# ngrabaskas/Torch-Automatic-Distributed-Neural-Network

Measured on AMD Instinct MI355X. Metric: samples/sec whole-node ResNet-50 DP + GPT-2 PP at 1/2/4/8 MI355X; scaling eff, higher is better.
Workload: dtype bf16

## Files before the change

madnn/models/resnet.py:

```python
from __future__ import annotations

import os
from typing import List, Optional, Type

import torch
from torch import nn

from ..nn.conv import FusedConv2d
from ..nn.norm import FusedBatchNorm2d as BN
from ..nn.norm import FusedGlobalAvgPool2d, FusedMaxPool2d
from ..ops import (batch_norm_add_bn_relu, bn_relu_conv1x1, bn_relu_conv1x1_epi_supported,
                   bn_relu_conv3x3, conv1x1_route,
                   bn_relu_conv3x3_supported, bn_relu_maxpool, bn_relu_maxpool_supported)

_FORK_DS = os.environ.get("MADNN_FORK_DOWNSAMPLE", "1") != "0"
_DUAL_BN = os.environ.get("MADNN_DUAL_BN", "1") != "0"
_DS_SUB = os.environ.get("MADNN_DS_SUB", "1") != "0"


def conv3x3(cin, cout, stride=1, groups=1, dilation=1):
    return FusedConv2d(cin, cout, 3, stride=stride, padding=dilation, groups=groups, bias=False, dilation=dilation)


def conv1x1(cin, cout, stride=1):
    return FusedConv2d(cin, cout, 1, stride=stride, bias=False)


class BasicBlock(nn.Module):
    expansion = 1

    def __init__(self, inplanes, planes, stride=1, downsample=None):
        super().__init__()
        self.conv1 = conv3x3(inplanes, planes, stride)
        self.bn1 = BN(planes)
        self.conv2 = conv3x3(planes, planes)
        self.bn2 = BN(planes)
        self.downsample = downsample

    def forward(self, x):
        idt = x if self.downsample is None else self.downsample(x)
        y, st = self.conv1(x, stats=True)
        out = self.bn1(y, relu=True, stats=st)
        y, st = self.conv2(out, stats=True)
        return self.bn2(y, residual=idt, relu=True, stats=st)


class Bottleneck(nn.Module):
    expansion = 4

    def __init__(self, inplanes, planes, stride=1, downsample=None):
        super().__init__()
        self.conv1 = conv1x1(inplanes, planes)
        self.bn1 = BN(planes)
        self.conv2 = conv3x3(planes, planes, stride)
        self.bn2 = BN(planes)
        self.conv3 = conv1x1(planes, planes * 4)
        self.bn3 = BN(planes * 4)
        self.downsample = downsample

    def forward(self, x):
        if self.downsample is None:
            y, st, idt = self.conv1(x, stats=True, fork=True)
            if isinstance(idt, torch.Tensor) and isinstance(self.bn3, BN) and self.conv1._k9(x) \
                    and conv1x1_route(x.size(1), self.conv1.weight.size(0))[1] == "k9":
                idt._madnn_defer_mask = True
        elif _FORK_DS:
            dual = self._dual_bn()
            sub = dual and _DS_SUB and isinstance(x, torch.Tensor) and self.downsample[0].subsampled_ok()
            y, st, xf = self.conv1(x, stats=True, fork=2 if sub else True)
            if dual:
                yd, std = (self.downsample[0].forward_subsampled(xf, stats=True) if sub
                           else self.downsample[0](xf, stats=True))
                y, st = self._bn1_conv2(y, st)
                y, st = self._bn2_conv3(y, st)
                return batch_norm_add_bn_relu(y, yd, self.bn3, self.downsample[1], st, std)
            idt = self.downsample(xf)
        else:
            idt = self.downsample(x)
            y, st = self.conv1(x, stats=True)
        y, st = self._bn1_conv2(y, st)
        y, st = self._bn2_conv3(y, st)
        return self.bn3(y, residual=idt, relu=True, stats=st)

    def _bn1_conv2(self, y, st):
        if isinstance(y, torch.Tensor) and isinstance(self.bn1, BN) and isinstance(self.conv2, FusedConv2d) \
                and self.conv2._k13(y) \
                and bn_relu_conv3x3_supported(y, self.bn1, self.conv2.weight):
            return bn_relu_conv3x3(y, self.bn1, self.conv2.weight, stats_in=st, stats=True)
        out = self.bn1(y, relu=True, stats=st)
        return self.conv2(out, stats=True)

    def _bn2_conv3(self, y, st):
        if isinstance(y, torch.Tensor) and isinstance(self.bn2, BN) and isinstance(self.conv3, FusedConv2d) \
                and self.conv3._k9(y) and bn_relu_conv1x1_epi_supported(y, self.bn2, self.conv3.weight):
            return bn_relu_conv1x1(y, self.bn2, self.conv3.weight, stats_in=st, stats=True)
        out = self.bn2(y, relu=True, stats=st)
        return self.conv3(out, stats=True)

    def _dual_bn(self) -> bool:
        ds = self.downsample
        return (_DUAL_BN and isinstance(ds, nn.Sequential) and len(ds) == 2
                and isinstance(ds[0], FusedConv2d) and isinstance(ds[1], BN) and isinstance(self.bn3, BN))


class ResNet(nn.Module):
# ... 80 lines not shown
```

madnn/ops/__init__.py:

```python
from __future__ import annotations

import os
import threading
from pathlib import Path
from typing import Optional, Sequence

import torch
import torch.nn.functional as F

from . import reference

HERE = Path(__file__).resolve().parent
_KERNELS = HERE / "_madnn_kernels.so"
_lock = threading.Lock()
_loaded = {"kernels": False, "error": None}


def kernels_path() -> Path:
    return _KERNELS


class StaleKernelsError(RuntimeError):
    """The in-tree kernel library was built from different sources than the tree holds."""

# ... 188 lines not shown
def _attach(t: torch.Tensor, name: str, value) -> None:
    setattr(t, name, (value, t._version))


def _attached(t: Optional[torch.Tensor], name: str, strict: bool = False):
    if t is None:
        return None
    rec = getattr(t, name, None)
    if rec is None and t._base is not None and t.numel() == t._base.numel():
        rec = getattr(t._base, name, None)
    if rec is None:
        return None
    value, version = rec
    if t._version != version:
        if strict:
            raise RuntimeError(f"madnn: gradient carrying {name} was modified in place after it was produced "
                               "(a second consumer's gradient accumulated into it); disable the deferral "
                               "(MADNN_DEFER_RES_MASK=0) for this model")
        return None
    return value


class _BNFn(torch.autograd.Function):
    @staticmethod
    def forward(ctx, x, weight, bias, residual, running_mean, running_var, nbt, training, momentum, eps, relu, stats):
        y, mean, invstd, scale, shift, mask = torch.ops.madnn.bn_fwd(x, residual, weight, bias, running_mean,
                                                                      running_var, nbt, bool(training),
                                                                      float(momentum), float(eps), bool(relu),
                                                                      stats if training else None)
        ctx.save_for_backward(x, mask, weight, mean, invstd, scale, shift)
        ctx.relu = relu
        ctx.has_res = residual is not None
        ctx.has_w = weight is not None
        ctx.defer = (DEFER_RES_MASK and relu and residual is not None and mask.numel() > 0
                     and getattr(residual, "_madnn_defer_mask", False))
        return y

    @staticmethod
    def backward(ctx, dy):
        x, mask, weight, mean, invstd, scale, shift = ctx.saved_tensors
        need_w = ctx.has_w and (ctx.needs_input_grad[1] or ctx.needs_input_grad[2])
        defer = ctx.defer and dy.dtype == x.dtype and dy.stride() == x.stride()
        dx, dw, db, dres = torch.ops.madnn.bn_bwd(dy, x, mask if mask.numel() else None, ctx.has_res, weight,
                                                  mean, invstd, scale, shift, ctx.relu, need_w, not defer)
        if defer:
            dres = dy.view_as(dy)
# ... 474 lines not shown


def bn_relu_conv1x1(y: torch.Tensor, bn, w: torch.Tensor, *, stats_in: Optional[torch.Tensor] = None,
                    stats: bool = False):
    if bn_relu_conv1x1_epi_supported(y, bn, w):
        _need_native("bn_relu_conv1x1")
        out, part = _BNReluConv1x1EpiFn.apply(y, w, bn.weight, bn.bias, bn, stats_in, stats)
        return (out, part if part.numel() else None) if stats else out
    a = bn(y, relu=True, stats=stats_in) if _is_fused_bn(bn) else torch.relu(bn(y))
    if conv1x1_supported(a, w):
        return conv1x1(a, w, stats=stats)
    out = torch.nn.functional.conv2d(a, w.view(w.size(0), -1, 1, 1)) if a.dim() == 4 else torch.mm(
        a, w.reshape(w.size(0), -1).t())
    return (out, None) if stats else out


def bn_relu_conv1x1_epi_supported(y: torch.Tensor, bn, w: torch.Tensor) -> bool:
    return (_BN_DGRAD_EPI and isinstance(y, torch.Tensor) and bn.training and bn.track_running_stats
            and bn.affine and bn.momentum is not None and bn.weight.dtype == torch.float32
            and conv1x1_supported(y, w) and bn_supported(y, bn.weight)
            and conv1x1_route(y.size(1), w.size(0))[1] == "k9")


class _BNReluMaxPoolFn(torch.autograd.Function):

    @staticmethod
    def forward(ctx, y, bn_w, bn_b, bn, stats_in, p):
        mean, invstd, scale, shift = torch.ops.madnn.bn_coef(y, bn_w, bn_b, bn.running_mean, bn.running_var,
                                                             bn.num_batches_tracked, float(bn.momentum),
                                                             float(bn.eps), stats_in)
        out, arg = torch.ops.madnn.pool_bn_fwd(y, scale, shift, int(p))
        ctx.save_for_backward(y, arg, bn_w, mean, invstd, scale, shift)
        ctx.p = int(p)
        return out

    @staticmethod
    def backward(ctx, dp):
        y, arg, bn_w, mean, invstd, scale, shift = ctx.saved_tensors
        dy, dw, db = torch.ops.madnn.pool_bn_bwd(dp, arg, y, bn_w, mean, invstd, scale, shift, ctx.p)
        return dy, dw, db, None, None, None


def bn_relu_maxpool_supported(y: torch.Tensor, bn, pool) -> bool:
    def pair(v):
        return tuple(v) if isinstance(v, (tuple, list)) else (v, v)
    return (_POOL_BN and isinstance(y, torch.Tensor) and y.device.type == "cuda" and y.dtype == torch.bfloat16 and y.dim() == 4
# ... 806 lines not shown
```

madnn/ops/csrc/binding.cpp:

```cpp
#include <torch/library.h>
#include <ATen/ATen.h>
#include <ATen/hip/impl/HIPGuardImplMasqueradingAsCUDA.h>
#include <ATen/hip/impl/HIPStreamMasqueradingAsCUDA.h>
#include <hip/hip_runtime.h>

#include <vector>

#include "attn.h"

extern "C" {
hipError_t madnn_bucket_pack(void* const*, const int64_t*, const int64_t*, int, void*, int, int, float, hipStream_t);
hipError_t madnn_bucket_unpack(void* const*, const int64_t*, const int64_t*, int, void*, int, int, float, hipStream_t);
hipError_t madnn_flat_scale_cast(const void*, void*, int64_t, int, int, float, hipStream_t);
hipError_t madnn_sgd_step(float*, const void*, int, float*, void*, int, int64_t, float, float, float, float, int, int,
                          float, const float*, hipStream_t);
hipError_t madnn_adam_step(float*, const void*, int, float*, float*, void*, int, int64_t, float, float, float, float,
                           float, int, float, float, float, const float*, hipStream_t);
int madnn_sqnorm_grid(int64_t);
hipError_t madnn_sqnorm_partial(const void*, int, int64_t, float, float*, int, hipStream_t);
hipError_t madnn_norm_finalize(const float*, int, float, float*, hipStream_t);
hipError_t madnn_norm_fwd(const void*, const void*, const void*, const void*, void*, void*, float*, float*, int64_t,
                          int, float, int, int, int, hipStream_t);
int64_t madnn_norm_bwd_workspace(int64_t, int);
hipError_t madnn_norm_bwd(const void*, const void*, const void*, const float*, const float*, const void*, void*, void*,
// ... 53 lines not shown
int64_t madnn_conv1x1_wgrad_ws(int64_t, int64_t, int64_t);
hipError_t madnn_conv1x1_wgrad(const void*, const void*, void*, int, float*, int64_t, int64_t, int64_t, hipStream_t);
hipError_t madnn_bn_coef(const void*, int64_t, int, float, float, const float*, const float*, float*, float*, int64_t*,
                         float*, float*, float*, float*, float*, const float*, int, hipStream_t);
int madnn_stem_supported(int, int);
int madnn_stem_stat_rows(int, int, int);
hipError_t madnn_stem_fwd(const void*, const void*, void*, float*, int, int, int, hipStream_t);
int64_t madnn_stem_wgrad_ws(int, int, int);
hipError_t madnn_stem_wgrad(const void*, const void*, float*, float*, int, int, int, hipStream_t);
int madnn_gemm_supported(int64_t, int64_t, int64_t, int64_t, int64_t);
int madnn_conv3x3_supported(int, int, int, int);
int madnn_conv3x3_stat_rows(int64_t);
hipError_t madnn_conv3x3_fwd(const void*, const void*, void*, float*, int, int, int, int, int, hipStream_t);
int madnn_conv3x3_s2_supported(int, int, int, int);
int madnn_conv3x3_s2_stat_rows(int, int, int);
hipError_t madnn_conv3x3_fwd_s2(const void*, const void*, void*, float*, int, int, int, int, int, hipStream_t);
int64_t madnn_conv3x3_wgrad_ws(int, int, int, int, int);
hipError_t madnn_conv3x3_fwd_bnb(const void*, const void*, void*, float*, const void*, const float*, const float*, int,
                                 int, int, int, int, hipStream_t);
hipError_t madnn_bn_bwd_ext(const void*, const void*, void*, int64_t, int, int, const float*, const float*,
                            const float*, const float*, const float*, float*, float*, float*, const float*, int, float*,
                            hipStream_t);
int madnn_bn_prereduce_floats(int);
hipError_t madnn_conv3x3_wgrad(const void*, const void*, float*, void*, int, int, int, int, int, int, hipStream_t);
hipError_t madnn_linear_fwd(const void*, const void*, const void*, int, const void*, void*, void*, int, int64_t,
                            int64_t, int64_t, hipStream_t);
hipError_t madnn_linear_dgrad(const void*, const void*, const void*, void*, int64_t, int64_t, int64_t, hipStream_t);
int madnn_wgrad_splits(int64_t, int64_t, int64_t);
hipError_t madnn_linear_wgrad4h(const void*, const void*, void*, float*, int, int, int64_t, int64_t, int64_t,
                                hipStream_t);
hipError_t madnn_linear_wgrad4(const void*, const void*, void*, float*, int, int, int64_t, int64_t, int64_t,
                               hipStream_t);
hipError_t madnn_linear_wgrad(const void*, const void*, void*, float*, int, int, int64_t, int64_t, int64_t,
                              hipStream_t);
int madnn_gemmp_supported(int64_t, int64_t, int64_t, int);
hipError_t madnn_linear_fwd_p(const void*, const void*, const void*, int, void*, void*, int, int64_t, int64_t,
                              int64_t, hipStream_t);
hipError_t madnn_linear_dgrad_p(const void*, const void*, const void*, void*, float*, int64_t, int64_t, int64_t, int,
                                hipStream_t);
hipError_t madnn_colsum_finalize(const float*, int, int64_t, void*, int, hipStream_t);
hipError_t madnn_hwq_wait(const int*, int, int64_t, int*, hipStream_t);
hipError_t madnn_hwq_set(int*, int, hipStream_t);
hipError_t madnn_hwq_batch(const int*, const int*, int, int*, int*, int, int64_t, int*, const int*, hipStream_t);
hipError_t madnn_hwq_spin(int64_t, hipStream_t);
}

// ... 468 lines not shown
                         const c10::optional<at::Tensor>& resmask) {
  const int64_t cout = dy.size(1), cin = w.numel() / std::max<int64_t>(cout, 1);
  const int64_t M = conv_rows(dy, cout, "dy");
  conv_check_w(w, cout, cin);
  at::hip::HIPGuardMasqueradingAsCUDA guard(dy.device());
  at::Tensor dx = conv_out_like(dy, cin);
  const bool has_res = res.has_value() && res->defined();
  if (has_res) {
    TORCH_CHECK(conv_rows(*res, cin, "res") == M && res->dim() == dy.dim(), "conv1x1_dgrad: residual layout");
  }
  const bool has_mask = resmask.has_value() && resmask->defined();
  if (has_mask) {
    TORCH_CHECK(has_res && resmask->scalar_type() == at::kByte && resmask->is_contiguous() &&
                    resmask->numel() == M * cin / 8, "conv1x1_dgrad: resmask must be a uint8 bit mask over res");
  }
  check(madnn_conv1x1_dgrad(dy.data_ptr(), w.data_ptr(), dx.data_ptr(), has_res ? res->data_ptr() : nullptr, M, cin,
                            cout, nullptr, nullptr, nullptr, nullptr, cur_stream(dy),
                            has_mask ? resmask->data_ptr<uint8_t>() : nullptr),
        "conv1x1_dgrad");
  return dx;
}

std::tuple<at::Tensor, at::Tensor> conv1x1_dgrad_bnb(const at::Tensor& dy, const at::Tensor& w, const at::Tensor& bny,
                                                     const at::Tensor& scale, const at::Tensor& shift) {
  const int64_t cout = dy.size(1), cin = w.numel() / std::max<int64_t>(cout, 1);
  const int64_t M = conv_rows(dy, cout, "dy");
  conv_check_w(w, cout, cin);
  TORCH_CHECK(conv_rows(bny, cin, "bny") == M && bny.dim() == dy.dim(), "conv1x1_dgrad_bnb: bny layout");
  TORCH_CHECK(scale.numel() == cin && shift.numel() == cin && scale.scalar_type() == at::kFloat &&
                  shift.scalar_type() == at::kFloat && scale.is_contiguous() && shift.is_contiguous(),
              "conv1x1_dgrad_bnb: fp32 [Cin] scale / shift");
  at::hip::HIPGuardMasqueradingAsCUDA guard(dy.device());
  at::Tensor dx = conv_out_like(dy, cin);
  at::Tensor part = at::empty({madnn_conv1x1_dgrad_rows(M, cin, cout), 2, cin}, dy.options().dtype(at::kFloat));
  check(madnn_conv1x1_dgrad(dy.data_ptr(), w.data_ptr(), dx.data_ptr(), nullptr, M, cin, cout, bny.data_ptr(),
                            scale.data_ptr<float>(), shift.data_ptr<float>(), part.data_ptr<float>(), cur_stream(dy)),
        "conv1x1_dgrad_bnb");
  return {dx, part};
}

at::Tensor conv1x1_wgrad(const at::Tensor& dy, const at::Tensor& x, bool out_bf16) {
  const int64_t cout = dy.size(1), cin = x.size(1);
  const int64_t M = conv_rows(x, cin, "x");
  TORCH_CHECK(conv_rows(dy, cout, "dy") == M && dy.dim() == x.dim(), "conv1x1_wgrad: dy / x pixel mismatch");
  TORCH_CHECK(madnn_conv1x1_supported(cin, cout), "conv1x1: channels must be multiples of 64");
  at::hip::HIPGuardMasqueradingAsCUDA guard(x.device());
  at::Tensor dw = at::empty({cout, cin}, x.options().dtype(out_bf16 ? at::kBFloat16 : at::kFloat));
  at::Tensor ws = at::empty({madnn_conv1x1_wgrad_ws(M, cin, cout)}, x.options().dtype(at::kFloat));
  check(madnn_conv1x1_wgrad(dy.data_ptr(), x.data_ptr(), dw.data_ptr(), out_bf16 ? 1 : 0, ws.data_ptr<float>(), M, cin,
                            cout, cur_stream(x)),
        "conv1x1_wgrad");
  return dw;
}

void gemm_check(const at::Tensor& t, const char* name) {
  check_dev(t, name);
  TORCH_CHECK(t.scalar_type() == at::kBFloat16, "linear: ", name, " must be bf16");
  TORCH_CHECK(t.is_contiguous(), "linear: ", name, " must be contiguous");
  TORCH_CHECK(reinterpret_cast<uintptr_t>(t.data_ptr()) % 16 == 0, "linear: ", name, " must be 16-B aligned");
}

// ... 728 lines not shown
      "xent_bwd(Tensor logits, Tensor targets, Tensor lse, bool shift, int V, int ignore_index, Tensor gscale) -> "
      "Tensor");
  m.def(
      "xent_fused(Tensor logits, Tensor targets, bool shift, int V, int ignore_index, Tensor gscale) -> "
      "(Tensor, Tensor)");
  m.def("xent_rescale(Tensor(a!) grad, Tensor g) -> ()");
  m.def(
      "bn_bwd(Tensor dy, Tensor x, Tensor? mask, bool has_res, Tensor? w, Tensor save_mean, Tensor save_invstd, "
      "Tensor scale, Tensor shift, bool relu, bool need_wgrad, bool write_dres=True) -> (Tensor, Tensor, Tensor, Tensor)");
  m.def(
      "bn_fwd_dual(Tensor x, Tensor r, Tensor? w, Tensor? b, Tensor(a!)? run_mean, Tensor(b!)? run_var, "
      "Tensor(c!)? nbt, float momentum, float eps, Tensor? partial, Tensor? w_r, Tensor? b_r, "
      "Tensor(d!)? run_mean_r, Tensor(e!)? run_var_r, Tensor(f!)? nbt_r, float momentum_r, float eps_r, "
      "Tensor? partial_r) -> Tensor[]");
  m.def(
      "bn_bwd_dual(Tensor dy, Tensor x, Tensor r, Tensor mask, Tensor? w, Tensor save_mean, Tensor save_invstd, "
      "Tensor? w_r, Tensor save_mean_r, Tensor save_invstd_r) -> Tensor[]");
  m.def("attn_fwd(Tensor q, Tensor k, Tensor v, bool causal, float scale) -> (Tensor, Tensor)");
  m.def(
      "attn_bwd(Tensor dout, Tensor q, Tensor k, Tensor v, Tensor o, Tensor lse, Tensor(a!) dq, Tensor(b!) dk, "
      "Tensor(c!) dv, bool causal, float scale, Tensor(d!)? colsum=None) -> ()");
  m.def("conv1x1_fwd(Tensor x, Tensor w, bool stats) -> (Tensor, Tensor)");
  m.def("conv1x1_dgrad(Tensor dy, Tensor w, Tensor? res=None, Tensor? resmask=None) -> Tensor");
  m.def("conv1x1_dgrad_bnb(Tensor dy, Tensor w, Tensor bny, Tensor scale, Tensor shift) -> (Tensor, Tensor)");
  m.def(
      "conv3x3_fwd_bnb(Tensor x, Tensor w, Tensor bny, Tensor scale, Tensor shift) -> (Tensor, Tensor)");
  m.def(
      "bn_bwd_ext(Tensor dy, Tensor x, Tensor? w, Tensor save_mean, Tensor save_invstd, Tensor scale, Tensor shift, "
      "Tensor partial, bool relu) -> (Tensor, Tensor, Tensor)");
  m.def("conv1x1_wgrad(Tensor dy, Tensor x, bool out_bf16=False) -> Tensor");
  m.def(
      "bn_coef(Tensor x, Tensor? w, Tensor? b, Tensor(a!)? run_mean, Tensor(b!)? run_var, Tensor(c!)? nbt, "
      "float momentum, float eps, Tensor? partial=None) -> Tensor[]");
  m.def("stem_fwd(Tensor x, Tensor wp, bool stats) -> (Tensor, Tensor)");
  m.def("linear_fwd(Tensor x, Tensor w, Tensor? bias, Tensor? res, int act, bool save_aux) -> (Tensor, Tensor)");
  m.def("linear_dgrad(Tensor dy, Tensor w, Tensor? res, bool accumulate) -> Tensor");
  m.def("linear_wgrad(Tensor dy, Tensor x, Tensor? out, bool accumulate, int splits) -> Tensor");
  m.def("linear_wgrad4(Tensor dy, Tensor x, Tensor? out, bool accumulate, int splits) -> Tensor");
  m.def("linear_wgrad4h(Tensor dy, Tensor x, Tensor? out, bool accumulate, int splits) -> Tensor");
  m.def("wgrad_splits(int M, int N, int K) -> int", &wgrad_splits);
  m.def("gemmp_supported(int I, int J, int K, bool has_bias) -> bool", &gemmp_supported);
  m.def("linear_fwd_p(Tensor x, Tensor w, Tensor? bias, int act) -> (Tensor, Tensor)");
  m.def("linear_dgrad_p(Tensor dy, Tensor w, Tensor? pre, ScalarType bias_dtype, int gelu_kind=1) -> (Tensor, Tensor)");
  m.def("conv3x3_fwd(Tensor x, Tensor w, bool stats) -> (Tensor, Tensor)");
  m.def("conv3x3_fwd_s2(Tensor x, Tensor w, bool stats) -> (Tensor, Tensor)");
  m.def("conv3x3_wgrad(Tensor dy, Tensor x, bool out_bf16) -> Tensor");
  m.def("stem_wgrad(Tensor dy, Tensor x) -> Tensor");
// ... 21 lines not shown
      "Tensor? dscale) -> ()");
  m.def("grad_norm(Tensor[] flats, float max_norm, float scale) -> Tensor");
  m.def("norm_fwd(Tensor x, Tensor? res, Tensor w, Tensor? b, float eps, bool rms) -> (Tensor, Tensor, Tensor, Tensor)");
  m.def(
      "norm_bwd(Tensor dy, Tensor x, Tensor w, Tensor mean, Tensor rstd, Tensor? dres, bool rms, bool has_bias, "
      "bool colsum=False, bool colsum_bf16=False) -> (Tensor, Tensor, Tensor, Tensor)");
}

TORCH_LIBRARY_IMPL(madnn, CUDA, m) {
  m.impl("bucket_pack", bucket_pack);
  m.impl("bucket_unpack", bucket_unpack);
  m.impl("flat_scale_cast", flat_scale_cast);
  m.impl("sgd_step", sgd_step);
  m.impl("adam_step", adam_step);
  m.impl("grad_norm", grad_norm);
  m.impl("norm_fwd", norm_fwd);
  m.impl("norm_bwd", norm_bwd);
  m.impl("bn_fwd", bn_fwd);
  m.impl("bn_bwd", bn_bwd);
  m.impl("bn_fwd_dual", bn_fwd_dual);
  m.impl("bn_coef", bn_coef);
  m.impl("conv3x3_fwd_bnb", conv3x3_fwd_bnb);
  m.impl("conv1x1_dgrad_bnb", conv1x1_dgrad_bnb);
  m.impl("bn_bwd_ext", bn_bwd_ext);
  m.impl("bn_bwd_dual", bn_bwd_dual);
  m.impl("xent_fwd", xent_fwd);
  m.impl("xent_bwd", xent_bwd);
  m.impl("xent_fused", xent_fused);
  m.impl("xent_rescale", xent_rescale);
  m.impl("maxpool_fwd", maxpool_fwd);
  m.impl("pool_bn_fwd", pool_bn_fwd);
  m.impl("pool_bn_bwd", pool_bn_bwd);
  m.impl("bias_grad", bias_grad);
  m.impl("gelu_fwd", gelu_fwd);
  m.impl("rope_qkv_", rope_qkv_);
  m.impl("rope_qkv", rope_qkv);
  m.impl("swiglu_fwd", swiglu_fwd);
  m.impl("swiglu_bwd", swiglu_bwd);
  m.impl("attn_fwd", attn_fwd);
  m.impl("attn_bwd", attn_bwd);
  m.impl("maxpool_bwd", maxpool_bwd);
  m.impl("conv1x1_fwd", conv1x1_fwd);
  m.impl("conv1x1_dgrad", conv1x1_dgrad);
  m.impl("conv1x1_wgrad", conv1x1_wgrad);
  m.impl("stem_fwd", stem_fwd);
  m.impl("stem_wgrad", stem_wgrad);
// ... 16 lines not shown
```

madnn/ops/csrc/bn.hip:

```cpp
#include <type_traits>

#include "common.h"

namespace madnn {

constexpr int kBnThreads = 256;
constexpr int kFinSlices = 32;

struct BnGeom {
  int tpr, rpi;
};

struct BnTune {
  int reverse = 1;
  int wg_per_cu = 3;
  int hoist = 1;
  int partials_per_cu = 2;
};
inline BnTune& bn_tune() {
  static BnTune t;
  return t;
}
inline int bn_walk_flags() { return (bn_tune().reverse ? 1 : 0) | (bn_tune().hoist ? 0 : 2); }

// ... 424 lines not shown
  __syncthreads();
  if (ls == 0 && c < C) {
    s = q = 0.f;
    for (int k = 0; k < kFinSlices; ++k) {
      s += red[0][k][lc];
      q += red[1][k][lc];
    }
    out[((int64_t)blockIdx.y * 2) * C + c] = s;
    out[((int64_t)blockIdx.y * 2 + 1) * C + c] = q;
  }
}

inline const float* prereduce(const float* part, int& G, int C, int& pstride, int& qoff, float* scratch,
                              hipStream_t stream) {
  if (G < kPreMinRows || scratch == nullptr || scratch == part) return part;
  hipLaunchKernelGGL(partial_prereduce_kernel, dim3((C + 31) / 32, kPreS), dim3(32 * kFinSlices), 0, stream, part, G,
                     C, pstride, qoff, scratch);
  G = kPreS;
  pstride = 2 * C;
  qoff = C;
  return scratch;
}

static int bn_grid_rows(int64_t M, int C) {
  const BnGeom g = bn_geom(C);
  const int64_t cap = (int64_t)bn_tune().partials_per_cu * kNumCU;
  int64_t iters = (M + g.rpi - 1) / g.rpi;
  return (int)(iters < cap ? (iters < 1 ? 1 : iters) : cap);
}

}

#define MADNN_BN_VARIANT(relu, res, RELU, RES, ...)                              \
  if (relu && res) { constexpr bool RELU = true, RES = true; __VA_ARGS__; }      \
  else if (relu) { constexpr bool RELU = true, RES = false; __VA_ARGS__; }       \
  else if (res) { constexpr bool RELU = false, RES = true; __VA_ARGS__; }        \
  else { constexpr bool RELU = false, RES = false; __VA_ARGS__; }

extern "C" {

int madnn_bn_tune(int key, int value) {
  int* f = key == 0   ? &madnn::bn_tune().reverse
           : key == 1 ? &madnn::bn_tune().wg_per_cu
           : key == 2 ? &madnn::bn_tune().hoist
           : key == 4 ? &madnn::bn_tune().partials_per_cu
                      : nullptr;
  if (f == nullptr) return -1;
  const int old = *f;
  if (value >= 0)
    *f = key == 1 ? (value < 1 ? 1 : value)
         : key == 4 ? (value < 1 ? 1 : value > 8 ? 8 : value)
                    : (value != 0);
  return old;
}

int madnn_bn_supported(int C) { return (C % 8 == 0 && C >= 8 && C <= 2048) ? 1 : 0; }

int madnn_bn_partial_rows(int64_t M, int C) { return madnn::bn_grid_rows(M, C); }

int madnn_bn_prereduce_floats(int C) { return madnn::kPreS * 2 * C; }

hipError_t madnn_bn_fwd(const void* x, const void* res, void* y, unsigned char* mask, int64_t M, int C, int xdt,
                        int relu, int training, float eps, float momentum, const float* w, const float* b,
                        float* run_mean, float* run_var, int64_t* nbt, float* save_mean, float* save_invstd,
                        float* scale, float* shift, float* workspace, const float* ext_partial, int ext_rows,
                        hipStream_t stream) {
  using namespace madnn;
  if (!madnn_bn_supported(C)) return hipErrorInvalidValue;
  if (M <= 0) return hipSuccess;
  int G = bn_grid_rows(M, C);
  const BnGeom g = bn_geom(C);
  const size_t lds = g.rpi > 1 ? (size_t)g.rpi * 2 * C * sizeof(float) : 0;
  if (training) {
    const float* part = workspace;
// ... 170 lines not shown
                            const float* save_mean, const float* save_invstd, const float* scale, const float* shift,
                            float* dw, float* db, float* coef, const float* partial, int G, float* scratch,
                            hipStream_t stream) {
  using namespace madnn;
  if (!madnn_bn_supported(C) || partial == nullptr || G <= 0) return hipErrorInvalidValue;
  if (M <= 0) return hipSuccess;
  int ps = 2 * C, qo = C;
  const float* part = prereduce(partial, G, C, ps, qo, scratch, stream);
  MADNN_HIP_CHECK(hipGetLastError());
  hipLaunchKernelGGL(bn_bwd_finalize_kernel, dim3((C + 31) / 32), dim3(32 * kFinSlices), 0, stream, part, G, C, ps,
                     qo, M, w, save_mean, save_invstd, dw, db, coef, coef + C, coef + 2 * C);
  MADNN_HIP_CHECK(hipGetLastError());
  const int64_t total = M * C;
  const int grid = stream_grid(total, 256 * 8, bn_tune().wg_per_cu * kNumCU);
  if (relu) {
    hipLaunchKernelGGL((bn_bwd_apply_kernel<kBF16, true, false>), dim3(grid), dim3(256), 0, stream, dy, x, nullptr,
                       scale, shift, coef, coef + C, coef + 2 * C, dx, nullptr, total, C, bn_walk_flags());
  } else {
    hipLaunchKernelGGL((bn_bwd_apply_kernel<kBF16, false, false>), dim3(grid), dim3(256), 0, stream, dy, x, nullptr,
                       scale, shift, coef, coef + C, coef + 2 * C, dx, nullptr, total, C, bn_walk_flags());
  }
  return hipGetLastError();
}
}
```

madnn/ops/csrc/conv.hip:

```cpp
#include "mfma.h"

namespace madnn {
namespace conv {

using namespace mf;

constexpr int kThreads = 256;
constexpr int kBK = 64;
constexpr int kTargetWG = 2 * kNumCU;

struct Tune {
  int fwd_wg = kTargetWG;
  int wgrad_wg = 2 * kNumCU;
  int xcd = 1;
};
inline Tune& tune() {
  static Tune t;
  return t;
}

enum Mode : int { kStoreT = 0, kSplit = 1 };

struct GemmArgs {
  const uint16_t* a;
// ... 380 lines not shown

hipError_t madnn_conv1x1_dgrad(const void* dy, const void* w, void* dx, const void* res, int64_t M, int64_t cin,
                               int64_t cout, const void* bny, const float* bnsc, const float* bnsh, float* partial,
                               hipStream_t s, const unsigned char* resmask) {
  if (!madnn_conv1x1_supported(cin, cout)) return hipErrorInvalidValue;
  if (M <= 0) return hipSuccess;
  GemmArgs p{};
  p.a = static_cast<const uint16_t*>(w);
  p.lda = cin;
  p.b = static_cast<const uint16_t*>(dy);
  p.ldb = cout;
  p.out = dx;
  p.res = static_cast<const uint16_t*>(res);
  p.resmask = res != nullptr ? resmask : nullptr;
  p.xcd = tune().xcd;
  p.ldo = cin;
  p.I = cin;
  p.J = M;
  p.K = cout;
  const bool wide = cin % 128 == 0;
  plan_persistent(p, M, wide ? 128 : 64, cin, cout);
  const int grid = p.i_tiles * p.j_groups;
  if (bny != nullptr) {
    if (partial == nullptr || bnsc == nullptr || bnsh == nullptr || res != nullptr) return hipErrorInvalidValue;
    p.bny = static_cast<const uint16_t*>(bny);
    p.bnsc = bnsc;
    p.bnsh = bnsh;
    p.stats = partial;
    return wide ? launch<true, false, 128, 128, kStoreT, false, true>(p, grid, s)
                : launch<true, false, 64, 128, kStoreT, false, true>(p, grid, s);
  }
  return wide ? launch<true, false, 128, 128, kStoreT, false>(p, grid, s)
              : launch<true, false, 64, 128, kStoreT, false>(p, grid, s);
}

int64_t madnn_conv1x1_wgrad_ws(int64_t M, int64_t cin, int64_t cout) {
  int bi, bj, kc;
  int64_t tiles, splits;
  wgrad_split(M, cin, cout, bi, bj, tiles, kc, splits);
  return splits * cin * cout;
}

hipError_t madnn_conv1x1_wgrad(const void* dy, const void* x, void* dw, int dw_bf16, float* ws, int64_t M, int64_t cin,
                               int64_t cout, hipStream_t s) {
  if (!madnn_conv1x1_supported(cin, cout)) return hipErrorInvalidValue;
  if (M <= 0) return hipMemsetAsync(dw, 0, (size_t)(cin * cout) * (dw_bf16 ? 2 : 4), s);
  GemmArgs p{};
// ... 37 lines not shown
```

madnn/ops/reference.py:

```python
from __future__ import annotations

import math
from typing import Optional, Sequence

import torch


def is_dense(t: torch.Tensor) -> bool:
    expected = 1
    for d in sorted(range(t.dim()), key=lambda d: t.stride(d)):
        if t.size(d) == 1:
            continue
        if t.stride(d) != expected:
            return False
        expected *= t.size(d)
    return True


def _flat_view(t: torch.Tensor) -> torch.Tensor:
    if t.is_contiguous():
        return t.reshape(-1)
    if not is_dense(t):
        raise ValueError("bucket tensors must be non-overlapping and dense")
    perm = sorted(range(t.dim()), key=lambda d: -t.stride(d))
# ... 80 lines not shown
    if bias is not None:
        y = y + bias.float()
    y = y.to(x.dtype)
    return (y, s) if residual is not None else y


def batch_norm_act(x, weight, bias, running_mean, running_var, num_batches_tracked=None, *, training, momentum=0.1,
                   eps=1e-5, relu=False, residual=None):
    import torch.nn.functional as F

    if training and num_batches_tracked is not None:
        num_batches_tracked.add_(1)
        if momentum is None:
            momentum = 1.0 / float(num_batches_tracked)
    y = F.batch_norm(x, running_mean, running_var, weight, bias, training, momentum if momentum is not None else 0.0,
                     eps)
    if residual is not None:
        y = y + residual
    if relu:
        y = torch.relu(y)
    return y


def cross_entropy(logits, targets, *, shift=False, vocab=None, ignore_index=-100):
    import torch.nn.functional as F

    v = vocab or logits.size(-1)
    if shift:
        logits, targets = logits[:, :-1], targets[:, 1:]
    return F.cross_entropy(logits[..., :v].reshape(-1, v).float(), targets.reshape(-1), ignore_index=ignore_index)


def attention(q, k, v, *, causal=True, scale=None):
    import torch.nn.functional as F

    h, hkv = q.size(2), k.size(2)
    o = F.scaled_dot_product_attention(q.transpose(1, 2), k.transpose(1, 2), v.transpose(1, 2),
                                       is_causal=causal, scale=scale, enable_gqa=h != hkv)
    return o.transpose(1, 2).contiguous()
```

Measured before the change: 13070.

## Fold bn3 backward into conv3 1x1 via Gram-matrix algebra for identity bottlenecks

Adds a fused conv1x1+BN+residual+ReLU autograd path for non-downsample bottleneck blocks. Its backward does not materialise the conv output. The BN backward is rewritten algebraically using the input Gram matrix, column sums and folded weights (Wp, Q, q0), so the BN-backward pass over the wide conv3 output is skipped and dgrad is fused with the bn2 backward. It needs extra small GEMMs (gram, Q) and a bf16 rounding-error correction. It applies only above a size threshold, which trades memory traffic on large activations for added compute and numerical risk.

```diff
diff --git a/madnn/models/resnet.py b/madnn/models/resnet.py
--- a/madnn/models/resnet.py
+++ b/madnn/models/resnet.py
@@ -10,7 +10,7 @@
 from ..nn.norm import FusedBatchNorm2d as BN
 from ..nn.norm import FusedGlobalAvgPool2d, FusedMaxPool2d
 from ..ops import (batch_norm_add_bn_relu, bn_relu_conv1x1, bn_relu_conv1x1_epi_supported,
-                   bn_relu_conv3x3, conv1x1_route,
+                   bn_relu_conv3x3, conv1x1_bn_add_relu, conv1x1_bn_add_relu_supported, conv1x1_route,
                    bn_relu_conv3x3_supported, bn_relu_maxpool, bn_relu_maxpool_supported)
 
 _FORK_DS = os.environ.get("MADNN_FORK_DOWNSAMPLE", "1") != "0"
@@ -46,6 +46,7 @@
 
 
 class Bottleneck(nn.Module):
+
     expansion = 4
 
     def __init__(self, inplanes, planes, stride=1, downsample=None):
@@ -79,8 +80,23 @@
             idt = self.downsample(x)
             y, st = self.conv1(x, stats=True)
         y, st = self._bn1_conv2(y, st)
+        if self.downsample is None:
+            out = self._conv3_bn3_folded(y, st, idt)
+            if out is not None:
+                return out
         y, st = self._bn2_conv3(y, st)
         return self.bn3(y, residual=idt, relu=True, stats=st)
+
+    def _conv3_bn3_folded(self, y, st, idt):
+        if not (isinstance(y, torch.Tensor) and isinstance(self.bn2, BN) and isinstance(self.conv3, FusedConv2d)
+                and self.conv3._k9(y)):
+            return None
+        w = self.conv3.weight
+        if conv1x1_bn_add_relu_supported(y, w, self.bn3, idt, bn2=self.bn2):
+            return conv1x1_bn_add_relu(y, w, self.bn3, idt, bn2=self.bn2, stats_in=st)
+        if conv1x1_bn_add_relu_supported(y, w, self.bn3, idt):
+            return conv1x1_bn_add_relu(self.bn2(y, relu=True, stats=st), w, self.bn3, idt)
+        return None
 
     def _bn1_conv2(self, y, st):
         if isinstance(y, torch.Tensor) and isinstance(self.bn1, BN) and isinstance(self.conv2, FusedConv2d) \
diff --git a/madnn/ops/__init__.py b/madnn/ops/__init__.py
--- a/madnn/ops/__init__.py
+++ b/madnn/ops/__init__.py
@@ -234,6 +234,7 @@
 
 
 class _BNFn(torch.autograd.Function):
+
     @staticmethod
     def forward(ctx, x, weight, bias, residual, running_mean, running_var, nbt, training, momentum, eps, relu, stats):
         y, mean, invstd, scale, shift, mask = torch.ops.madnn.bn_fwd(x, residual, weight, bias, running_mean,
@@ -754,6 +755,100 @@
             and conv1x1_route(y.size(1), w.size(0))[1] == "k9")
 
 
+BN3_FOLD = os.environ.get("MADNN_BN3_FOLD", "1") != "0"
+BN3_FOLD_MIN = int(os.environ.get("MADNN_BN3_FOLD_MIN", str(800_000_000)))
+
+
+class _Conv1x1BNAddReluFn(torch.autograd.Function):
+
+    @staticmethod
+    def forward(ctx, x, w, bn3_w, bn3_b, idt, bn3, bn2_w, bn2_b, bn2, stats_in):
+        bn2_saved = ()
+        if bn2 is not None:
+            a, mean2, invstd2, scale2, shift2, _ = torch.ops.madnn.bn_fwd(
+                x, None, bn2_w, bn2_b, bn2.running_mean, bn2.running_var, bn2.num_batches_tracked, True,
+                float(bn2.momentum), float(bn2.eps), True, stats_in)
+            bn2_saved = (x, bn2_w, mean2, invstd2, scale2, shift2)
+        else:
+            a = x
+        fwd, dgrad, _ = conv1x1_route(a.size(1), w.size(0))
+        if fwd == "k9":
+            x3, part = torch.ops.madnn.conv1x1_fwd(a, w, True)
+        else:
+            x3 = torch.nn.functional.conv2d(a, w) if a.dim() == 4 else torch.mm(a, w.reshape(w.size(0), -1).t())
+            part = None
+        out, mean, invstd, _, _, mask = torch.ops.madnn.bn_fwd(
+            x3, idt, bn3_w, bn3_b, bn3.running_mean, bn3.running_var, bn3.num_batches_tracked, True,
+            float(bn3.momentum), float(bn3.eps), True, part if part is not None and part.numel() else None)
+        ctx.save_for_backward(a, w, mask, mean, invstd, bn3_w, *bn2_saved)
+        ctx.route = dgrad
+        return out
+
+    @staticmethod
+    def backward(ctx, dy):
+        a, w, mask, mean, invstd, bn3_w, *bn2_saved = ctx.saved_tensors
+        dgrad = ctx.route
+        dy = _nhwc(dy.to(a.dtype))
+        g, s1 = torch.ops.madnn.bn_mask_colsum(dy, mask)
+        p = _fold_wgrad(g, a, w)
+        a2 = _rows(a)
+        gram = torch.ops.madnn.conv1x1_wgrad(a, a, False)
+        sa = torch.ops.madnn.bias_grad(a2, None, torch.float32, 1)[0]
+        dw, wp, q, q0, dg, db = torch.ops.madnn.bn_fold_finalize(s1, p, w, gram, sa, bn3_w, mean, invstd,
+                                                                 a2.size(0))
+        t = torch.empty_like(a)
+        torch.addmm(q0.to(a.dtype), a2, q, out=_rows(t))
+        dbw = dbb = None
+        if bn2_saved:
+            y, bn2_w, mean2, invstd2, scale2, shift2 = bn2_saved
+            da, part = torch.ops.madnn.conv1x1_dgrad_bnb(g, wp, y, scale2, shift2, t)
+            dx, dbw, dbb = torch.ops.madnn.bn_bwd_ext(da, y, bn2_w, mean2, invstd2, scale2, shift2, part, True)
+        elif dgrad == "k9":
+            dx = torch.ops.madnn.conv1x1_dgrad(g, wp, t, None)
+        else:
+            _rows(t).addmm_(_rows(g), wp)
+            dx = t
+        return dx, dw, dg, db, g, None, dbw, dbb, None, None
+
+
+def _fold_wgrad(g: torch.Tensor, a: torch.Tensor, w: torch.Tensor) -> torch.Tensor:
+    dr, xr = _rows(g), _rows(a)
+    choice = _WGRAD_CHOICE.get(("conv1x1", dr.shape[0], dr.shape[1], xr.shape[1]))
+    if WGRAD in ("k12", "k12w", "k12wh"):
+        choice = WGRAD
+    if choice in ("k12", "k12w", "k12wh") and w.dtype == torch.bfloat16 and _wgrad_k12_ok(
+            dr, xr, torch.empty(0, dtype=w.dtype, device=w.device)) and (choice != "k12wh" or dr.shape[0] % 128 == 0):
+        op = {"k12": torch.ops.madnn.linear_wgrad, "k12w": torch.ops.madnn.linear_wgrad4,
+              "k12wh": torch.ops.madnn.linear_wgrad4h}[choice]
+        return op(dr, xr, None, False, 0).view(w.shape)
+    return _k9_wgrad(g, a, w)
+
+
+def conv1x1_bn_add_relu_supported(x: torch.Tensor, w: torch.Tensor, bn3, idt: torch.Tensor, bn2=None) -> bool:
+    def ok(m):
+        return (_is_fused_bn(m) and m.training and m.track_running_stats and m.affine and m.momentum is not None
+                and m.weight.dtype == torch.float32)
+    if not (BN3_FOLD and isinstance(x, torch.Tensor) and isinstance(idt, torch.Tensor)):
+        return False
+    if not (ok(bn3) and conv1x1_supported(x, w) and x.dim() == 4 and w.size(0) <= 2048 and load_kernels()):
+        return False
+    if bn2 is not None and not bn_relu_conv1x1_epi_supported(x, bn2, w):
+        return False
+    n, _, h, wd = x.shape
+    if n * h * wd * w.size(0) < BN3_FOLD_MIN:
+        return False
+    return (idt.shape == (n, w.size(0), h, wd) and idt.dtype == x.dtype and idt.device == x.device
+            and idt.is_contiguous(memory_format=torch.channels_last))
+
+
+def conv1x1_bn_add_relu(x: torch.Tensor, w: torch.Tensor, bn3, idt: torch.Tensor, bn2=None,
+                        stats_in: Optional[torch.Tensor] = None) -> torch.Tensor:
+    _need_native("conv1x1_bn_add_relu")
+    if bn2 is None:
+        return _Conv1x1BNAddReluFn.apply(x, w, bn3.weight, bn3.bias, idt, bn3, None, None, None, None)
+    return _Conv1x1BNAddReluFn.apply(x, w, bn3.weight, bn3.bias, idt, bn3, bn2.weight, bn2.bias, bn2, stats_in)
+
+
 class _BNReluMaxPoolFn(torch.autograd.Function):
 
     @staticmethod
diff --git a/madnn/ops/csrc/binding.cpp b/madnn/ops/csrc/binding.cpp
--- a/madnn/ops/csrc/binding.cpp
+++ b/madnn/ops/csrc/binding.cpp
@@ -99,6 +99,11 @@
                             const float*, const float*, const float*, float*, float*, float*, const float*, int, float*,
                             hipStream_t);
 int madnn_bn_prereduce_floats(int);
+int madnn_bn_mask_rows(int64_t, int);
+hipError_t madnn_bn_mask_colsum(const void*, const unsigned char*, void*, int64_t, int, int, float*, hipStream_t);
+hipError_t madnn_bn_fold_finalize(const float*, int, int, int, const void*, const void*, const float*, const float*,
+                                  int64_t, const float*, const float*, const float*, float*, float*, float*, void*,
+                                  void*, void*, float*, float*, hipStream_t);
 hipError_t madnn_conv3x3_wgrad(const void*, const void*, float*, void*, int, int, int, int, int, int, hipStream_t);
 hipError_t madnn_linear_fwd(const void*, const void*, const void*, int, const void*, void*, void*, int, int64_t,
                             int64_t, int64_t, hipStream_t);
@@ -613,7 +618,8 @@
 }
 
 std::tuple<at::Tensor, at::Tensor> conv1x1_dgrad_bnb(const at::Tensor& dy, const at::Tensor& w, const at::Tensor& bny,
-                                                     const at::Tensor& scale, const at::Tensor& shift) {
+                                                     const at::Tensor& scale, const at::Tensor& shift,
+                                                     const c10::optional<at::Tensor>& res) {
   const int64_t cout = dy.size(1), cin = w.numel() / std::max<int64_t>(cout, 1);
   const int64_t M = conv_rows(dy, cout, "dy");
   conv_check_w(w, cout, cin);
@@ -621,13 +627,66 @@
   TORCH_CHECK(scale.numel() == cin && shift.numel() == cin && scale.scalar_type() == at::kFloat &&
                   shift.scalar_type() == at::kFloat && scale.is_contiguous() && shift.is_contiguous(),
               "conv1x1_dgrad_bnb: fp32 [Cin] scale / shift");
+  const bool has_res = res.has_value() && res->defined();
+  if (has_res) {
+    TORCH_CHECK(conv_rows(*res, cin, "res") == M && res->dim() == dy.dim(), "conv1x1_dgrad_bnb: residual layout");
+  }
   at::hip::HIPGuardMasqueradingAsCUDA guard(dy.device());
   at::Tensor dx = conv_out_like(dy, cin);
   at::Tensor part = at::empty({madnn_conv1x1_dgrad_rows(M, cin, cout), 2, cin}, dy.options().dtype(at::kFloat));
-  check(madnn_conv1x1_dgrad(dy.data_ptr(), w.data_ptr(), dx.data_ptr(), nullptr, M, cin, cout, bny.data_ptr(),
-                            scale.data_ptr<float>(), shift.data_ptr<float>(), part.data_ptr<float>(), cur_stream(dy)),
+  check(madnn_conv1x1_dgrad(dy.data_ptr(), w.data_ptr(), dx.data_ptr(), has_res ? res->data_ptr() : nullptr, M, cin,
+                            cout, bny.data_ptr(), scale.data_ptr<float>(), shift.data_ptr<float>(),
+                            part.data_ptr<float>(), cur_stream(dy)),
         "conv1x1_dgrad_bnb");
   return {dx, part};
+}
+
+std::tuple<at::Tensor, at::Tensor> bn_mask_colsum(const at::Tensor& dy, const at::Tensor& mask) {
+  check_dev(dy, "dy");
+  const int64_t C = dy.size(1);
+  TORCH_CHECK(madnn_bn_supported((int)C), "bn kernel needs C % 8 == 0 and C <= 2048, got ", C);
+  const int64_t M = bn_rows(dy, C);
+  TORCH_CHECK(mask.scalar_type() == at::kByte && mask.is_contiguous() && mask.numel() == dy.numel() / 8,
+              "bn_mask_colsum: mask must be a uint8 bit mask over dy");
+  at::hip::HIPGuardMasqueradingAsCUDA guard(dy.device());
+  at::Tensor g = at::empty_like(dy);
+  at::Tensor part = at::empty({M > 0 ? (int64_t)madnn_bn_mask_rows(M, (int)C) : 0, C}, dy.options().dtype(at::kFloat));
+  check(madnn_bn_mask_colsum(dy.data_ptr(), mask.data_ptr<uint8_t>(), g.data_ptr(), M, (int)C, dt_code(dy),
+                             part.data_ptr<float>(), cur_stream(dy)),
+        "bn_mask_colsum");
+  return {g, part};
+}
+
+std::vector<at::Tensor> bn_fold_finalize(const at::Tensor& part, const at::Tensor& p, const at::Tensor& w,
+                                         const at::Tensor& gram, const at::Tensor& sa,
+                                         const c10::optional<at::Tensor>& bn_w, const at::Tensor& save_mean,
+                                         const at::Tensor& save_invstd, int64_t M) {
+  check_dev(w, "w");
+  const int64_t C = w.size(0), K = w.numel() / std::max<int64_t>(C, 1);
+  conv_check_w(w, C, K);
+  TORCH_CHECK(madnn_bn_supported((int)C), "bn_fold_finalize: unsupported channel count ", C);
+  TORCH_CHECK(p.scalar_type() == at::kBFloat16 && p.numel() == C * K && p.size(0) == C && p.stride(0) == K &&
+                  p.stride(1) == 1 && p.is_cuda(),
+              "bn_fold_finalize: p must be bf16 [C, K] with contiguous rows");
+  TORCH_CHECK(part.scalar_type() == at::kFloat && part.is_contiguous() && part.dim() == 2 && part.size(1) == C &&
+                  part.size(0) > 0,
+              "bn_fold_finalize: partial column sums must be fp32 [rows, C]");
+  TORCH_CHECK(gram.scalar_type() == at::kFloat && gram.is_contiguous() && gram.numel() == K * K &&
+                  sa.scalar_type() == at::kFloat && sa.is_contiguous() && sa.numel() == K,
+              "bn_fold_finalize: gram fp32 [K, K], sa fp32 [K]");
+  TORCH_CHECK(save_mean.numel() == C && save_invstd.numel() == C && M > 0, "bn_fold_finalize: statistics");
+  at::hip::HIPGuardMasqueradingAsCUDA guard(w.device());
+  auto fo = w.options().dtype(at::kFloat);
+  at::Tensor dW = at::empty_like(w), Wp = at::empty({C, K}, w.options()), Q = at::empty({K, K}, w.options());
+  at::Tensor q0 = at::empty({K}, fo), dg = at::empty({C}, fo), dbt = at::empty({C}, fo), coef = at::empty({3 * C}, fo);
+  at::Tensor qerr = at::empty({K, K}, fo);
+  check(madnn_bn_fold_finalize(part.data_ptr<float>(), (int)part.size(0), (int)C, (int)K, p.data_ptr(), w.data_ptr(),
+                               gram.data_ptr<float>(), sa.data_ptr<float>(), M, optf(bn_w), optf(save_mean),
+                               optf(save_invstd), dg.data_ptr<float>(), dbt.data_ptr<float>(), coef.data_ptr<float>(),
+                               dW.data_ptr(), Wp.data_ptr(), Q.data_ptr(), q0.data_ptr<float>(), qerr.data_ptr<float>(),
+                               cur_stream(w)),
+        "bn_fold_finalize");
+  return {dW, Wp, Q, q0, dg, dbt};
 }
 
 at::Tensor conv1x1_wgrad(const at::Tensor& dy, const at::Tensor& x, bool out_bf16) {
@@ -1402,7 +1461,12 @@
       "Tensor(c!) dv, bool causal, float scale, Tensor(d!)? colsum=None) -> ()");
   m.def("conv1x1_fwd(Tensor x, Tensor w, bool stats) -> (Tensor, Tensor)");
   m.def("conv1x1_dgrad(Tensor dy, Tensor w, Tensor? res=None, Tensor? resmask=None) -> Tensor");
-  m.def("conv1x1_dgrad_bnb(Tensor dy, Tensor w, Tensor bny, Tensor scale, Tensor shift) -> (Tensor, Tensor)");
+  m.def("conv1x1_dgrad_bnb(Tensor dy, Tensor w, Tensor bny, Tensor scale, Tensor shift, Tensor? res=None) -> "
+        "(Tensor, Tensor)");
+  m.def("bn_mask_colsum(Tensor dy, Tensor mask) -> (Tensor, Tensor)");
+  m.def(
+      "bn_fold_finalize(Tensor part, Tensor p, Tensor w, Tensor gram, Tensor sa, Tensor? bn_w, Tensor save_mean, "
+      "Tensor save_invstd, int M) -> Tensor[]");
   m.def(
       "conv3x3_fwd_bnb(Tensor x, Tensor w, Tensor bny, Tensor scale, Tensor shift) -> (Tensor, Tensor)");
   m.def(
@@ -1470,6 +1534,8 @@
   m.impl("bn_coef", bn_coef);
   m.impl("conv3x3_fwd_bnb", conv3x3_fwd_bnb);
   m.impl("conv1x1_dgrad_bnb", conv1x1_dgrad_bnb);
+  m.impl("bn_mask_colsum", bn_mask_colsum);
+  m.impl("bn_fold_finalize", bn_fold_finalize);
   m.impl("bn_bwd_ext", bn_bwd_ext);
   m.impl("bn_bwd_dual", bn_bwd_dual);
   m.impl("xent_fwd", xent_fwd);
diff --git a/madnn/ops/csrc/bn.hip b/madnn/ops/csrc/bn.hip
--- a/madnn/ops/csrc/bn.hip
+++ b/madnn/ops/csrc/bn.hip
@@ -470,11 +470,223 @@
   return scratch;
 }
 
-static int bn_grid_rows(int64_t M, int C) {
+static int bn_grid_rows(int64_t M, int C, int per_cu = 0) {
   const BnGeom g = bn_geom(C);
-  const int64_t cap = (int64_t)bn_tune().partials_per_cu * kNumCU;
+  const int64_t cap = (int64_t)(per_cu > 0 ? per_cu : bn_tune().partials_per_cu) * kNumCU;
   int64_t iters = (M + g.rpi - 1) / g.rpi;
   return (int)(iters < cap ? (iters < 1 ? 1 : iters) : cap);
+}
+
+
+template <int XDT>
+__global__ __launch_bounds__(kBnThreads) void bn_mask_colsum_kernel(const void* __restrict__ dy,
+                                                                     const unsigned char* __restrict__ mask,
+                                                                     void* __restrict__ gout, int64_t M, int C,
+                                                                     float* __restrict__ partial) {
+  extern __shared__ __attribute__((aligned(16))) float slab[];
+  const BnGeom g = bn_geom(C);
+  const int t = threadIdx.x;
+  const int cg = t % g.tpr;
+  const int rs = t / g.tpr;
+  const bool active = rs < g.rpi;
+  float sg[8];
+#pragma unroll
+  for (int j = 0; j < 8; ++j) sg[j] = 0.f;
+  if (active) {
+    const int64_t step = (int64_t)gridDim.x * g.rpi;
+    int64_t r = (int64_t)blockIdx.x * g.rpi + rs;
+    auto body = [&](int64_t i, float (&dv)[8], unsigned bits) {
+#pragma unroll
+      for (int j = 0; j < 8; ++j) {
+        dv[j] = ((bits >> j) & 1u) ? dv[j] : 0.f;
+        sg[j] += dv[j];
+      }
+      store8<XDT>(gout, i, dv);
+    };
+    for (; r + step < M; r += 2 * step) {
+      float dv[2][8];
+      unsigned mb[2];
+#pragma unroll
+      for (int u = 0; u < 2; ++u) {
+        load8<XDT>(dy, (r + u * step) * C + cg * 8, dv[u]);
+        mb[u] = mask[((r + u * step) * C + cg * 8) >> 3];
+      }
+      body(r * C + cg * 8, dv[0], mb[0]);
+      body((r + step) * C + cg * 8, dv[1], mb[1]);
+    }
+    for (; r < M; r += step) {
+      float dv[8];
+      load8<XDT>(dy, r * C + cg * 8, dv);
+      body(r * C + cg * 8, dv, mask[(r * C + cg * 8) >> 3]);
+    }
+  }
+  if (g.rpi == 1) {
+    if (active) store8<kF32>(partial, (int64_t)blockIdx.x * C + cg * 8, sg);
+    return;
+  }
+  if (active) {
+#pragma unroll
+    for (int j = 0; j < 8; ++j) slab[rs * C + cg * 8 + j] = sg[j];
+  }
+  __syncthreads();
+  for (int c = t; c < C; c += kBnThreads) {
+    float a = 0.f;
+    for (int r = 0; r < g.rpi; ++r) a += slab[r * C + c];
+    partial[(int64_t)blockIdx.x * C + c] = a;
+  }
+}
+
+__global__ __launch_bounds__(1024) void fold_coef_kernel(const float* __restrict__ partial, int G, int C, int K,
+                                                         const uint16_t* __restrict__ P,
+                                                         const uint16_t* __restrict__ W, int64_t M,
+                                                         const float* __restrict__ w, const float* __restrict__ mean,
+                                                         const float* __restrict__ invstd, float* __restrict__ dw,
+                                                         float* __restrict__ db, float* __restrict__ ca,
+                                                         float* __restrict__ cb, float* __restrict__ cc) {
+  __shared__ double red[2][kFinSlices][33];
+  const int lc = threadIdx.x & 31, ls = threadIdx.x >> 5;
+  const int c = blockIdx.x * 32 + lc;
+  double s = 0.0, q = 0.0;
+  if (c < C)
+    for (int k = ls; k < G; k += kFinSlices) s += partial[(int64_t)k * C + c];
+  const int row = blockIdx.x * 32 + ls;
+  if (row < C)
+    for (int k = lc; k < K; k += 32)
+      q += (double)(bf16_to_f32(P[(int64_t)row * K + k]) * bf16_to_f32(W[(int64_t)row * K + k]));
+  red[0][ls][lc] = s;
+  red[1][ls][lc] = q;
+  __syncthreads();
+  if (ls == 0 && c < C) {
+    s = q = 0.0;
+    for (int k = 0; k < kFinSlices; ++k) {
+      s += red[0][k][lc];
+      q += red[1][lc][k];
+    }
+    const double mu = mean[c], is = invstd[c];
+    const double dbeta = s;
+    const double dgamma = is * (q - mu * s);
+    if (dw) dw[c] = (float)dgamma;
+    if (db) db[c] = (float)dbeta;
+    const double wc = w ? w[c] : 1.0;
+    const double A = wc * is;
+    const double k2 = dbeta / (double)M, k3 = dgamma / (double)M;
+    ca[c] = (float)A;
+    cb[c] = (float)(-A * is * k3);
+    cc[c] = (float)(A * (is * k3 * mu - k2));
+  }
+}
+
+constexpr int kFoldT = 64, kFoldK = 16;
+
+template <bool A_KFAST, class FA, class FB>
+__device__ __forceinline__ void fold_tile_gemm(int i0, int j0, int red, FA la, FB lb, float (&acc)[4][4]) {
+  __shared__ __attribute__((aligned(16))) float As[kFoldK][kFoldT + 4];
+  __shared__ __attribute__((aligned(16))) float Bs[kFoldK][kFoldT + 4];
+  const int tx = threadIdx.x & 15, ty = threadIdx.x >> 4;
+  for (int k0 = 0; k0 < red; k0 += kFoldK) {
+#pragma unroll
+    for (int u = 0; u < kFoldK * kFoldT / 256; ++u) {
+      const int e = threadIdx.x + 256 * u;
+      const int ai = A_KFAST ? e / kFoldK : e % kFoldT, ak = A_KFAST ? e % kFoldK : e / kFoldT;
+      As[ak][ai] = la(i0 + ai, k0 + ak);
+      Bs[e / kFoldT][e % kFoldT] = lb(k0 + e / kFoldT, j0 + e % kFoldT);
+    }
+    __syncthreads();
+#pragma unroll
+    for (int kk = 0; kk < kFoldK; ++kk) {
+      float a[4], b[4];
+#pragma unroll
+      for (int r = 0; r < 4; ++r) {
+        a[r] = As[kk][4 * ty + r];
+        b[r] = Bs[kk][4 * tx + r];
+      }
+#pragma unroll
+      for (int r = 0; r < 4; ++r)
+#pragma unroll
+        for (int s = 0; s < 4; ++s) acc[r][s] += a[r] * b[s];
+    }
+    __syncthreads();
+  }
+}
+
+__device__ __forceinline__ void fold_store4(uint16_t* dst, const float (&v)[4]) {
+  uint2 o;
+  o.x = (unsigned)f32_to_bf16(v[0]) | ((unsigned)f32_to_bf16(v[1]) << 16);
+  o.y = (unsigned)f32_to_bf16(v[2]) | ((unsigned)f32_to_bf16(v[3]) << 16);
+  *reinterpret_cast<uint2*>(dst) = o;
+}
+
+__global__ __launch_bounds__(256) void fold_dw_kernel(const uint16_t* __restrict__ P, const uint16_t* __restrict__ W,
+                                                      const float* __restrict__ Gm, const float* __restrict__ sa,
+                                                      const float* __restrict__ ca, const float* __restrict__ cb,
+                                                      const float* __restrict__ cc, int K,
+                                                      uint16_t* __restrict__ dW, uint16_t* __restrict__ Wp) {
+  const int i0 = blockIdx.y * kFoldT, j0 = blockIdx.x * kFoldT;
+  float acc[4][4] = {};
+  fold_tile_gemm<true>(
+      i0, j0, K, [&](int c, int j) { return bf16_to_f32(W[(int64_t)c * K + j]); },
+      [&](int j, int k) { return Gm[(int64_t)j * K + k]; }, acc);
+  const int tx = threadIdx.x & 15, ty = threadIdx.x >> 4;
+  const int k = j0 + 4 * tx;
+#pragma unroll
+  for (int r = 0; r < 4; ++r) {
+    const int c = i0 + 4 * ty + r;
+    const float a = ca[c], b = cb[c], d = cc[c];
+    float o[4], wp[4];
+#pragma unroll
+    for (int s = 0; s < 4; ++s) {
+      o[s] = a * bf16_to_f32(P[(int64_t)c * K + k + s]) + b * acc[r][s] + d * sa[k + s];
+      wp[s] = a * bf16_to_f32(W[(int64_t)c * K + k + s]);
+    }
+    fold_store4(dW + (int64_t)c * K + k, o);
+    fold_store4(Wp + (int64_t)c * K + k, wp);
+  }
+}
+
+__global__ __launch_bounds__(256) void fold_q_kernel(const uint16_t* __restrict__ W, const float* __restrict__ cb,
+                                                     int C, int K, uint16_t* __restrict__ Q,
+                                                     float* __restrict__ Qerr) {
+  const int i0 = blockIdx.y * kFoldT, j0 = blockIdx.x * kFoldT;
+  float acc[4][4] = {};
+  fold_tile_gemm<false>(
+      i0, j0, C, [&](int k, int c) { return bf16_to_f32(W[(int64_t)c * K + k]) * cb[c]; },
+      [&](int c, int k) { return bf16_to_f32(W[(int64_t)c * K + k]); }, acc);
+  const int tx = threadIdx.x & 15, ty = threadIdx.x >> 4;
+#pragma unroll
+  for (int r = 0; r < 4; ++r) {
+    const int64_t o = (int64_t)(i0 + 4 * ty + r) * K + j0 + 4 * tx;
+    fold_store4(Q + o, acc[r]);
+#pragma unroll
+    for (int s = 0; s < 4; ++s) Qerr[o + s] = acc[r][s] - bf16_to_f32(f32_to_bf16(acc[r][s]));
+  }
+}
+
+__global__ __launch_bounds__(1024) void fold_q0_kernel(const uint16_t* __restrict__ W, const float* __restrict__ cc,
+                                                       const float* __restrict__ sa,
+                                                       const float* __restrict__ Qerr, int C, int K, int64_t M,
+                                                       float* __restrict__ q0) {
+  __shared__ float red[kFinSlices][33];
+  const int lc = threadIdx.x & 31, ls = threadIdx.x >> 5;
+  const int k = blockIdx.x * 32 + lc;
+  float s = 0.f;
+  if (k < K) {
+    for (int c = ls; c < C; c += kFinSlices) s += cc[c] * bf16_to_f32(W[(int64_t)c * K + k]);
+    float e = 0.f;
+    for (int j = ls; j < K; j += kFinSlices) e += sa[j] * Qerr[(int64_t)j * K + k];
+    s += e / (float)M;
+  }
+  red[ls][lc] = s;
+  __syncthreads();
+  if (ls == 0 && k < K) {
+    s = 0.f;
+    for (int i = 0; i < kFinSlices; ++i) s += red[i][lc];
+    q0[k] = s;
+  }
+}
+
+inline int& fold_mask_wg_per_cu() {
+  static int v = 3;
+  return v;
 }
 
 }
@@ -492,12 +704,13 @@
            : key == 1 ? &madnn::bn_tune().wg_per_cu
            : key == 2 ? &madnn::bn_tune().hoist
            : key == 4 ? &madnn::bn_tune().partials_per_cu
+           : key == 5 ? &madnn::fold_mask_wg_per_cu()
                       : nullptr;
   if (f == nullptr) return -1;
   const int old = *f;
   if (value >= 0)
     *f = key == 1 ? (value < 1 ? 1 : value)
-         : key == 4 ? (value < 1 ? 1 : value > 8 ? 8 : value)
+         : (key == 4 || key == 5) ? (value < 1 ? 1 : value > 8 ? 8 : value)
                     : (value != 0);
   return old;
 }
@@ -714,4 +927,46 @@
   }
   return hipGetLastError();
 }
-}
+
+int madnn_bn_mask_rows(int64_t M, int C) { return madnn::bn_grid_rows(M, C, madnn::fold_mask_wg_per_cu()); }
+
+hipError_t madnn_bn_mask_colsum(const void* dy, const unsigned char* mask, void* g, int64_t M, int C, int xdt,
+                                float* partial, hipStream_t stream) {
+  using namespace madnn;
+  if (!madnn_bn_supported(C) || mask == nullptr || g == dy) return hipErrorInvalidValue;
+  if (M <= 0) return hipSuccess;
+  const int G = madnn_bn_mask_rows(M, C);
+  const BnGeom geo = bn_geom(C);
+  const size_t lds = geo.rpi > 1 ? (size_t)geo.rpi * C * sizeof(float) : 0;
+  MADNN_DISPATCH_DT(xdt, XDT, {
+    hipLaunchKernelGGL((bn_mask_colsum_kernel<XDT>), dim3(G), dim3(kBnThreads), lds, stream, dy, mask, g, M, C,
+                       partial);
+  });
+  return hipGetLastError();
+}
+
+hipError_t madnn_bn_fold_finalize(const float* partial, int G, int C, int K, const void* P, const void* W,
+                                  const float* Gm, const float* sa, int64_t M, const float* w, const float* mean,
+                                  const float* invstd, float* dw, float* db, float* coef, void* dW, void* Wp, void* Q,
+                                  float* q0, float* qerr, hipStream_t stream) {
+  using namespace madnn;
+  if (!madnn_bn_supported(C) || C % kFoldT || K % kFoldT || K <= 0 || G <= 0 || M <= 0) return hipErrorInvalidValue;
+  const uint16_t* Pp = static_cast<const uint16_t*>(P);
+  const uint16_t* Wq = static_cast<const uint16_t*>(W);
+  float* ca = coef;
+  float* cb = coef + C;
+  float* cc = coef + 2 * C;
+  hipLaunchKernelGGL(fold_coef_kernel, dim3((C + 31) / 32), dim3(32 * kFinSlices), 0, stream, partial, G, C, K, Pp, Wq,
+                     M, w, mean, invstd, dw, db, ca, cb, cc);
+  MADNN_HIP_CHECK(hipGetLastError());
+  hipLaunchKernelGGL(fold_dw_kernel, dim3(K / kFoldT, C / kFoldT), dim3(256), 0, stream, Pp, Wq, Gm, sa, ca, cb, cc, K,
+                     static_cast<uint16_t*>(dW), static_cast<uint16_t*>(Wp));
+  MADNN_HIP_CHECK(hipGetLastError());
+  hipLaunchKernelGGL(fold_q_kernel, dim3(K / kFoldT, K / kFoldT), dim3(256), 0, stream, Wq, cb, C, K,
+                     static_cast<uint16_t*>(Q), qerr);
+  MADNN_HIP_CHECK(hipGetLastError());
+  hipLaunchKernelGGL(fold_q0_kernel, dim3((K + 31) / 32), dim3(32 * kFinSlices), 0, stream, Wq, cc, sa, qerr, C, K,
+                     M, q0);
+  return hipGetLastError();
+}
+}
diff --git a/madnn/ops/csrc/conv.hip b/madnn/ops/csrc/conv.hip
--- a/madnn/ops/csrc/conv.hip
+++ b/madnn/ops/csrc/conv.hip
@@ -426,7 +426,7 @@
   plan_persistent(p, M, wide ? 128 : 64, cin, cout);
   const int grid = p.i_tiles * p.j_groups;
   if (bny != nullptr) {
-    if (partial == nullptr || bnsc == nullptr || bnsh == nullptr || res != nullptr) return hipErrorInvalidValue;
+    if (partial == nullptr || bnsc == nullptr || bnsh == nullptr) return hipErrorInvalidValue;
     p.bny = static_cast<const uint16_t*>(bny);
     p.bnsc = bnsc;
     p.bnsh = bnsh;
diff --git a/madnn/ops/reference.py b/madnn/ops/reference.py
--- a/madnn/ops/reference.py
+++ b/madnn/ops/reference.py
@@ -126,6 +126,46 @@
     return y
 
 
+def bn3_fold_backward(a, w, gamma, mean, invstd, dy, keep):
+    m = a.shape[0]
+    g = dy * keep.to(dy.dtype)
+    p = g.t() @ a
+    s1 = g.sum(0)
+    s2 = (p * w).sum(1)
+    dbeta = s1
+    dgamma = invstd * (s2 - mean * s1)
+    amp = gamma * invstd
+    k2, k3 = dbeta / m, dgamma / m
+    ca, cb, cc = amp, -amp * invstd * k3, amp * (invstd * k3 * mean - k2)
+    gram, sa = a.t() @ a, a.sum(0)
+    dw = ca[:, None] * p + cb[:, None] * (w @ gram) + cc[:, None] * sa[None, :]
+    wp = ca[:, None] * w
+    q = w.t() @ (cb[:, None] * w)
+    q0 = cc @ w
+    da = g @ wp + a @ q + q0
+    return da, dw, dgamma, dbeta, g
+
+
+class _Conv1x1BNAddRelu(torch.autograd.Function):
+    @staticmethod
+    def forward(ctx, a, w, gamma, beta, res, eps):
+        x = a @ w.t()
+        mean = x.mean(0)
+        invstd = torch.rsqrt(x.var(0, unbiased=False) + eps)
+        z = (x - mean) * invstd * gamma + beta + res
+        ctx.save_for_backward(a, w, gamma, mean, invstd, z > 0)
+        return torch.relu(z)
+
+    @staticmethod
+    def backward(ctx, dy):
+        a, w, gamma, mean, invstd, keep = ctx.saved_tensors
+        return (*bn3_fold_backward(a, w, gamma, mean, invstd, dy, keep), None)
+
+
+def conv1x1_bn_add_relu(a, w, gamma, beta, res, eps=1e-5):
+    return _Conv1x1BNAddRelu.apply(a, w, gamma, beta, res, eps)
+
+
 def cross_entropy(logits, targets, *, shift=False, vocab=None, ignore_index=-100):
     import torch.nn.functional as F
 
```

Measured after the change: 13200, median of 6. About the same (+0.9%).
